# meta-pytorch/torchx

Hardware: AMD Instinct MI355X
Metric: tokens_per_second (higher is better)
Workload: dtype bf16; 1 GPU; model=llama3_8b, global_batch=4, seq_len=4096, parallelism=dp1

## Files before the change

torchx_amd/models/llama.py:

```python

from __future__ import annotations

from dataclasses import dataclass
from typing import Optional, Tuple

import torch
import torch.nn as nn

from torchx_amd import ops


@dataclass
class LlamaConfig:
    vocab_size: int = 128256
    hidden_size: int = 4096
    intermediate_size: int = 14336
    num_layers: int = 32
    num_heads: int = 32
    num_kv_heads: int = 8
    head_dim: int = 128
    max_seq_len: int = 8192
    rope_theta: float = 500000.0
    rms_eps: float = 1e-5
    tie_embeddings: bool = False

    @property
    def q_dim(self) -> int:
        return self.num_heads * self.head_dim

    @property
    def kv_dim(self) -> int:
        return self.num_kv_heads * self.head_dim


def llama3_8b() -> LlamaConfig:
    return LlamaConfig()


def llama_tiny(vocab: int = 512) -> LlamaConfig:
    return LlamaConfig(
        vocab_size=vocab, hidden_size=256, intermediate_size=512,
        num_layers=2, num_heads=4, num_kv_heads=2, head_dim=64,
        max_seq_len=256,
    )


def llama_gpu_tiny(vocab: int = 512) -> LlamaConfig:
    return LlamaConfig(
        vocab_size=vocab, hidden_size=2048, intermediate_size=4096,
        num_layers=2, num_heads=8, num_kv_heads=4, head_dim=128,
        max_seq_len=512,
    )


def _lin(mod: nn.Module, x: torch.Tensor) -> torch.Tensor:
    if type(mod) is nn.Linear and mod.bias is None and x.is_cuda:
        return ops.fast_linear(x, mod.weight)
    return mod(x)


def _new_linear(in_features: int, out_features: int,
                device: Optional[torch.device]) -> nn.Linear:
    if device is not None and torch.device(device).type == "cuda":
        return torch.nn.utils.skip_init(
            nn.Linear, in_features, out_features, bias=False,
            dtype=torch.bfloat16, device=device)
    return nn.Linear(in_features, out_features, bias=False,
                     dtype=torch.bfloat16)


class LlamaBlock(nn.Module):
    def __init__(self, cfg: LlamaConfig,
                 device: Optional[torch.device] = None):
        super().__init__()
        self.cfg = cfg
        h, qd, kvd = cfg.hidden_size, cfg.q_dim, cfg.kv_dim
        self.wqkv = _new_linear(h, qd + 2 * kvd, device)
        self.wo = _new_linear(qd, h, device)
        self.wgu = _new_linear(h, 2 * cfg.intermediate_size, device)
        self.wdown = _new_linear(cfg.intermediate_size, h, device)
        self.attn_norm = nn.Parameter(torch.ones(h, dtype=torch.bfloat16))
        self.mlp_norm = nn.Parameter(torch.ones(h, dtype=torch.bfloat16))

    def forward(self, x: torch.Tensor, cos: torch.Tensor,
                sin: torch.Tensor, delta: Optional[torch.Tensor] = None
                ) -> Tuple[torch.Tensor, torch.Tensor]:
        cfg = self.cfg
        B, S, H = x.shape
        if delta is None:
            xn = ops.rmsnorm(x, self.attn_norm, cfg.rms_eps)
        else:
            x, xn = ops.add_rmsnorm(x, delta, self.attn_norm, cfg.rms_eps)
        qkv = _lin(self.wqkv, xn)
        attn = ops.fused_attention_qkv(
            qkv, cos, sin, cfg.num_heads, cfg.num_kv_heads, causal=True
        )
        x, xn = ops.add_rmsnorm(
            x, _lin(self.wo, attn.reshape(B, S, cfg.q_dim)), self.mlp_norm,
            cfg.rms_eps)
        return x, _lin(self.wdown, ops.swiglu_packed(_lin(self.wgu, xn)))


class LlamaModel(nn.Module):

    def __init__(self, cfg: LlamaConfig, device: Optional[torch.device] = None):
        super().__init__()
        self.cfg = cfg
        factory = {"dtype": torch.bfloat16, "device": device}
        self.embed = nn.Embedding(cfg.vocab_size, cfg.hidden_size, **factory)
        self.blocks = nn.ModuleList(
            [LlamaBlock(cfg, device) for _ in range(cfg.num_layers)]
        )
        self.final_norm = nn.Parameter(
            torch.ones(cfg.hidden_size, dtype=torch.bfloat16)
        )
        self.lm_head = _new_linear(cfg.hidden_size, cfg.vocab_size, device)
        if cfg.tie_embeddings:
            self.lm_head.weight = self.embed.weight
        cos, sin = ops.rope_tables(cfg.max_seq_len, cfg.head_dim,
                                   cfg.rope_theta, device=device)
        self.register_buffer("rope_cos", cos, persistent=False)
        self.register_buffer("rope_sin", sin, persistent=False)
        if device is not None:
            self.to(device)
        self.apply(self._init_weights)

    def _init_weights(self, m: nn.Module) -> None:
        std = 0.02
        if isinstance(m, nn.Linear):
            nn.init.normal_(m.weight, mean=0.0, std=std)
        elif isinstance(m, nn.Embedding):
            nn.init.normal_(m.weight, mean=0.0, std=std)

    def forward_hidden(self, tokens: torch.Tensor) -> torch.Tensor:
        x = self.embed(tokens)
        cos, sin = self.rope_cos, self.rope_sin
        delta = None
        for blk in self.blocks:
            x, delta = blk(x, cos, sin, delta)
        if delta is None:
            return ops.rmsnorm(x, self.final_norm, self.cfg.rms_eps)
        return ops.add_rmsnorm(x, delta, self.final_norm,
                               self.cfg.rms_eps)[1]

    def forward(self, tokens: torch.Tensor,
                targets: Optional[torch.Tensor] = None) -> torch.Tensor:
        x = self.forward_hidden(tokens)
        if targets is None:
            return self.lm_head(x)
        return ops.fused_linear_cross_entropy(
            x, self.lm_head.weight, targets
        )

    def num_params(self) -> int:
        return sum(p.numel() for p in self.parameters())
```

torchx_amd/ops/__init__.py:

```python

from __future__ import annotations

import importlib.util
import math
from pathlib import Path
from typing import Optional, Tuple

import torch

from . import reference

_SO = Path(__file__).resolve().parent / "_hip_ops.so"
_hip = None
_load_err: Optional[str] = None


def _load():
    global _hip, _load_err
    if _hip is not None:
        return _hip
    if not _SO.exists():
        _load_err = f"{_SO} not built (run torchx_amd/ops/build.py)"
        return None
    try:
# ... 109 lines not shown
        return dx, None, None, None


def rope(x: torch.Tensor, cos: torch.Tensor, sin: torch.Tensor) -> torch.Tensor:
    heads = x.shape[2]
    if _on_gpu(x):
        return _RoPE.apply(x, cos, sin, heads)
    return reference.rope(x, cos, sin)




class _SwiGLU(torch.autograd.Function):
    @staticmethod
    def forward(ctx, g: torch.Tensor, u: torch.Tensor):
        ctx.save_for_backward(g, u)
        return hip_ops().swiglu_fwd(g.contiguous(), u.contiguous())

    @staticmethod
    def backward(ctx, dout: torch.Tensor):
        g, u = ctx.saved_tensors
        dg, du = hip_ops().swiglu_bwd(dout.contiguous(), g, u)
        return dg, du


def swiglu(g: torch.Tensor, u: torch.Tensor) -> torch.Tensor:
    if _on_gpu(g):
        return _SwiGLU.apply(g, u)
    return reference.swiglu(g, u)




class _CrossEntropy(torch.autograd.Function):
    @staticmethod
    def forward(ctx, logits: torch.Tensor, targets: torch.Tensor):
        V = logits.shape[-1]
        logits2d = logits.contiguous().view(-1, V)
        loss, lse = hip_ops().ce_fwd(logits2d, targets.contiguous().view(-1))
        ctx.save_for_backward(logits2d, targets, lse)
        ctx.orig_shape = logits.shape
        return loss.mean()

    @staticmethod
    def backward(ctx, gout: torch.Tensor):
        logits2d, targets, lse = ctx.saved_tensors
        T = logits2d.shape[0]
        gscale = (gout.float() / T).expand(T).contiguous()
        dlogits = hip_ops().ce_bwd(logits2d, targets.view(-1), lse, gscale)
        return dlogits.view(ctx.orig_shape), None


def cross_entropy(logits: torch.Tensor, targets: torch.Tensor) -> torch.Tensor:
    if _on_gpu(logits):
        return _CrossEntropy.apply(logits, targets)
    return reference.cross_entropy(logits, targets)




class _FusedLinearCE(torch.autograd.Function):
    @staticmethod
    def forward(ctx, x2: torch.Tensor, w: torch.Tensor,
                targets: torch.Tensor, chunk: int):
        hip = hip_ops()
        T, H = x2.shape
        dx = torch.empty_like(x2)
        single = T <= chunk
        dw_acc = None if single else torch.zeros_like(w, dtype=torch.float32)
        loss_sum = torch.zeros((), device=x2.device, dtype=torch.float32)
        inv_t = 1.0 / T
        gscale = torch.full((min(chunk, T),), inv_t, device=x2.device,
                            dtype=torch.float32)
        wt = (hip.transpose_bf16(w)
              if w.shape[0] % 64 == 0 and w.shape[1] % 64 == 0 else None)
        for s in range(0, T, chunk):
            e = min(T, s + chunk)
            x_c = x2[s:e]
            t_c = targets[s:e].contiguous()
            logits_c = x_c @ w.t()
            loss_c, lse_c = hip.ce_fwd(logits_c, t_c)
            loss_sum += loss_c.sum()
            dlog_c = hip.ce_bwd(logits_c, t_c, lse_c, gscale[:e - s])
            if wt is not None:
                torch.matmul(dlog_c, wt.t(), out=dx[s:e])
            else:
                torch.matmul(dlog_c, w, out=dx[s:e])
            if single:
                dw_acc = dlog_c.t() @ x_c
            else:
                dw_acc += dlog_c.t() @ x_c
        ctx.save_for_backward(dx, dw_acc)
        return loss_sum * inv_t

    @staticmethod
    def backward(ctx, gout: torch.Tensor):
        dx, dw_acc = ctx.saved_tensors
        if dw_acc.dtype == dx.dtype:
            dw = dw_acc * gout.to(dx.dtype)
        else:
            dw = (dw_acc * gout.to(torch.float32)).to(dx.dtype)
        dx = dx * gout.to(dx.dtype)
        return dx, dw, None, None


def fused_linear_cross_entropy(
    x: torch.Tensor, w: torch.Tensor, targets: torch.Tensor,
    chunk: int = 16384,
) -> torch.Tensor:
    H = x.shape[-1]
    x2 = x.reshape(-1, H)
    t = targets.reshape(-1)
    if _on_gpu(x):
        if torch.is_grad_enabled() and (x.requires_grad or w.requires_grad):
            return _FusedLinearCE.apply(x2.contiguous(), w, t, chunk)
        hip = hip_ops()
        x2 = x2.contiguous()
        T = x2.shape[0]
        loss_sum = torch.zeros((), device=x.device, dtype=torch.float32)
        for s in range(0, T, chunk):
            e = min(T, s + chunk)
            loss_c, _ = hip.ce_fwd(x2[s:e] @ w.t(), t[s:e].contiguous())
            loss_sum += loss_c.sum()
        return loss_sum / T
    return reference.cross_entropy(x2 @ w.t(), t)




class _FlashAttention(torch.autograd.Function):
    @staticmethod
    def forward(ctx, q: torch.Tensor, k: torch.Tensor, v: torch.Tensor,
                causal: bool, scale: float):
        o, lse = hip_ops().attn_fwd(
            q.contiguous(), k.contiguous(), v.contiguous(), scale, causal
        )
        ctx.save_for_backward(q, k, v, o, lse)
        ctx.causal = causal
        ctx.scale = scale
        return o

    @staticmethod
    def backward(ctx, dout: torch.Tensor):
        q, k, v, o, lse = ctx.saved_tensors
        dq, dk, dv = hip_ops().attn_bwd(
            q, k, v, o, dout.contiguous(), lse, ctx.scale, ctx.causal
        )
        return dq, dk, dv, None, None


def set_attn_bwd_dq_mode(mode: str) -> None:
    hip_ops().set_attn_bwd_dq_mode(mode)


def get_attn_bwd_dq_mode() -> str:
    return hip_ops().get_attn_bwd_dq_mode()


def set_attn_bwd_dkv_impl(impl: str) -> None:
    hip_ops().set_attn_bwd_dkv_impl(impl)


def get_attn_bwd_dkv_impl() -> str:
    return hip_ops().get_attn_bwd_dkv_impl()


def set_attn_fwd_map(name: str) -> None:
    hip_ops().set_attn_fwd_map(name)


def get_attn_fwd_map() -> str:
    return hip_ops().get_attn_fwd_map()


def flash_attention(
    q: torch.Tensor, k: torch.Tensor, v: torch.Tensor,
    causal: bool = True, scale: Optional[float] = None,
) -> torch.Tensor:
    if scale is None:
        scale = 1.0 / math.sqrt(q.shape[-1])
    if _on_gpu(q):
        return _FlashAttention.apply(q, k, v, causal, scale)
    return reference.attention(q, k, v, causal=causal, scale=scale)




def adamw_step(
    p32: torch.Tensor, p16: torch.Tensor, grad: torch.Tensor,
    m: torch.Tensor, v: torch.Tensor, *, lr: float, beta1: float = 0.9,
    beta2: float = 0.95, eps: float = 1e-8, weight_decay: float = 0.1,
    step: int = 1,
) -> None:
    if p32.is_cuda:
        hip_ops().adamw_step(p32, p16, grad, m, v, lr, beta1, beta2, eps,
                             weight_decay, step)
    else:
        reference.adamw_step(p32, p16, grad, m, v, lr=lr, beta1=beta1,
                             beta2=beta2, eps=eps, weight_decay=weight_decay,
                             step=step)


def mfma_probe(a: torch.Tensor, b: torch.Tensor) -> torch.Tensor:
    return hip_ops().mfma_probe(a, b)




class _FastLinear(torch.autograd.Function):
    @staticmethod
    def forward(ctx, x: torch.Tensor, w: torch.Tensor):
        ctx.save_for_backward(x, w)
        return x @ w.t()

    @staticmethod
    def backward(ctx, dy: torch.Tensor):
        x, w = ctx.saved_tensors
        hip = hip_ops()
        wt = hip.transpose_bf16(w)
        dy2 = dy.reshape(-1, dy.shape[-1]).contiguous()
        x2 = x.reshape(-1, x.shape[-1])
        dx = (dy2 @ wt.t()).view_as(x)
        M, N = dy2.shape
        via_t = N <= 8192 and M % 64 == 0 and N % 64 == 0
        wg = w.grad if w.is_leaf else None
        if wg is not None and wg.is_contiguous():
            a = hip.transpose_bf16(dy2) if via_t else dy2.t()
            if getattr(w, "_wgrad_fresh", False):
                torch.matmul(a, x2, out=wg)
                w._wgrad_fresh = False
            else:
                wg.addmm_(a, x2)
            from torchx_amd.parallel.ddp import grad_ready

            grad_ready(w)
            return dx, None
        dw = (hip.transpose_bf16(dy2) @ x2) if via_t else (dy2.t() @ x2)
        return dx, dw


def fast_linear(x: torch.Tensor, w: torch.Tensor) -> torch.Tensor:
    if (x.is_cuda and w.dtype == torch.bfloat16
            and w.shape[0] % 64 == 0 and w.shape[1] % 64 == 0):
        return _FastLinear.apply(x, w)
    return torch.nn.functional.linear(x, w)




class _FusedAttentionQKV(torch.autograd.Function):
    @staticmethod
    def forward(ctx, qkv: torch.Tensor, cos: torch.Tensor, sin: torch.Tensor,
                Hq: int, Hkv: int, causal: bool, scale: float):
        hip = hip_ops()
        roped = hip.rope_qkv(qkv.contiguous(), cos, sin, Hq, Hkv, 1.0, False)
        o, lse = hip.attn_fwd_qkv(roped, Hq, Hkv, scale, causal)
        ctx.save_for_backward(roped, o, lse, cos, sin)
        ctx.dims = (Hq, Hkv, causal, scale)
        return o

    @staticmethod
    def backward(ctx, dout: torch.Tensor):
        roped, o, lse, cos, sin = ctx.saved_tensors
        Hq, Hkv, causal, scale = ctx.dims
        hip = hip_ops()
        dqkv = hip.attn_bwd_qkv(roped, o, dout.contiguous(), lse, Hq, Hkv,
                                scale, causal)
        hip.rope_qkv(dqkv, cos, sin, Hq, Hkv, -1.0, True)
        return dqkv, None, None, None, None, None, None


def fused_attention_qkv(
    qkv: torch.Tensor, cos: torch.Tensor, sin: torch.Tensor,
    Hq: int, Hkv: int, causal: bool = True,
    scale: Optional[float] = None,
) -> torch.Tensor:
    D = qkv.shape[-1] // (Hq + 2 * Hkv)
    if scale is None:
        scale = 1.0 / math.sqrt(D)
    if _on_gpu(qkv):
        return _FusedAttentionQKV.apply(qkv, cos, sin, Hq, Hkv, causal, scale)
    B, S, _ = qkv.shape
    q, k, v = qkv.split([Hq * D, Hkv * D, Hkv * D], dim=-1)
    q = reference.rope(q.reshape(B, S, Hq, D), cos, sin)
    k = reference.rope(k.reshape(B, S, Hkv, D), cos, sin)
    return reference.attention(q, k, v.reshape(B, S, Hkv, D),
                               causal=causal, scale=scale)


class _SwiGLUPacked(torch.autograd.Function):
    @staticmethod
    def forward(ctx, gu: torch.Tensor):
        gu = gu.contiguous()
        ctx.save_for_backward(gu)
        return hip_ops().swiglu_gu_fwd(gu)

    @staticmethod
    def backward(ctx, dout: torch.Tensor):
        (gu,) = ctx.saved_tensors
        return hip_ops().swiglu_gu_bwd(dout.contiguous(), gu)


def swiglu_packed(gu: torch.Tensor) -> torch.Tensor:
    if _on_gpu(gu):
        return _SwiGLUPacked.apply(gu)
    g, u = gu.chunk(2, dim=-1)
    return reference.swiglu(g, u)




def decode_attention(q: torch.Tensor, kcache: torch.Tensor,
                     vcache: torch.Tensor, length: int,
                     scale: Optional[float] = None) -> torch.Tensor:
    if scale is None:
        scale = 1.0 / math.sqrt(q.shape[-1])
    if _on_gpu(q):
        return hip_ops().decode_attn(q.contiguous(), kcache, vcache,
                                     length, scale)
    return reference.decode_attention(q, kcache, vcache, length, scale)


def rmsnorm_res(x: torch.Tensor, res: Optional[torch.Tensor],
                w: torch.Tensor, eps: float = 1e-5):
    if _on_gpu(x):
        s, y = hip_ops().rmsnorm_res(x.contiguous(),
                                     res.contiguous() if res is not None
                                     else None, w.contiguous(), eps)
        return s, y
    s = x if res is None else (x + res)
    return s, reference.rmsnorm(s, w, eps)


def decode_rope_cache(qkv: torch.Tensor, kcache: torch.Tensor,
                      vcache: torch.Tensor, cos: torch.Tensor,
                      sin: torch.Tensor, pos,
                      num_heads: int) -> torch.Tensor:
    B = qkv.shape[0]
    Hkv, D = kcache.shape[2], kcache.shape[3]
    if _on_gpu(qkv):
        if isinstance(pos, torch.Tensor):
            return hip_ops().decode_rope_cache(qkv.contiguous(), kcache,
                                               vcache, cos, sin, 0, pos)
        return hip_ops().decode_rope_cache(qkv.contiguous(), kcache, vcache,
                                           cos, sin, int(pos), None)
    q, k, v = qkv.split([num_heads * D, Hkv * D, Hkv * D], dim=-1)
    q = q.reshape(B, 1, num_heads, D)
    k = k.reshape(B, 1, Hkv, D)
    v = v.reshape(B, 1, Hkv, D)
    if isinstance(pos, torch.Tensor) and pos.numel() > 1:
        outs = []
        for b in range(B):
            p = int(pos[b].item())
            cs, sn = cos[p:p + 1], sin[p:p + 1]
            outs.append(rope(q[b:b + 1].contiguous(), cs, sn))
            kcache[b, p:p + 1] = rope(k[b:b + 1].contiguous(), cs, sn)[0]
            vcache[b, p:p + 1] = v[b]
        return torch.cat(outs, dim=0).reshape(B, num_heads, D)
    p = int(pos.item()) if isinstance(pos, torch.Tensor) else int(pos)
    cs, sn = cos[p:p + 1], sin[p:p + 1]
    q = rope(q.contiguous(), cs, sn)
    k = rope(k.contiguous(), cs, sn)
    kcache[:, p:p + 1] = k
    vcache[:, p:p + 1] = v
    return q.reshape(B, num_heads, D)


def decode_linear_swiglu(x: torch.Tensor, w: torch.Tensor) -> torch.Tensor:
    x2 = x.reshape(-1, x.shape[-1])
    M, K = x2.shape
    if _on_gpu(x) and M <= 8 and K % 512 == 0 and w.shape[0] % 2 == 0 \
            and w.dtype == torch.bfloat16 and w.is_contiguous():
        out = hip_ops().gemv_swiglu_bf16(x2.contiguous(), w)
    else:
        gu = x2 @ w.t()
        g, u = gu.chunk(2, dim=-1)
        out = torch.nn.functional.silu(g.float()).to(u.dtype) * u
    return out.reshape(*x.shape[:-1], w.shape[0] // 2)


def decode_attention_dev(q: torch.Tensor, kcache: torch.Tensor,
                         vcache: torch.Tensor, pos: torch.Tensor,
                         scale: Optional[float] = None) -> torch.Tensor:
    if scale is None:
        scale = 1.0 / math.sqrt(q.shape[-1])
    if _on_gpu(q):
        return hip_ops().decode_attn_dev(q.contiguous(), kcache, vcache,
                                         pos.contiguous(), scale)
    if pos.numel() == 1:
        return reference.decode_attention(q, kcache, vcache,
# ... 162 lines not shown
```

torchx_amd/ops/csrc/bindings.cpp:

```cpp
#include <torch/extension.h>
#include <c10/hip/HIPStream.h>

#include <hip/hip_runtime.h>

extern "C" {
void rope_launch(const void*, void*, const void*, const void*, long, int, int,
                 int, float, hipStream_t);
void swiglu_fwd_launch(const void*, const void*, void*, long, hipStream_t);
void swiglu_bwd_launch(const void*, const void*, const void*, void*, void*,
                       long, hipStream_t);
void rmsnorm_fwd_launch(const void*, const void*, void*, void*, long, int,
                        float, hipStream_t);
void rmsnorm_bwd_launch(const void*, const void*, const void*, const void*,
                        const void*, void*, void*, void*, long, int,
                        hipStream_t);
long rmsnorm_bwd_dw_chunks(long);
void adamw_launch(void*, void*, const void*, void*, void*, long, float, float,
                  float, float, float, float, float, hipStream_t);
void ce_fwd_launch(const void*, const void*, void*, void*, long, int,
                   hipStream_t);
void ce_bwd_launch(const void*, const void*, const void*, const void*, void*,
                   long, int, hipStream_t);
void attn_fwd_launch(const void*, const void*, const void*, void*, void*, int,
                     int, int, int, float, int, long, long, hipStream_t);
void attn_bwd_launch(const void*, const void*, const void*, const void*,
                     const void*, const void*, void*, void*, void*, void*,
                     void*, int, int, int, int, float, int, long, long, long,
                     long, hipStream_t);
long attn_bwd_ds_bytes(int, int, int, int);
int attn_bwd_dkv_impl_get();
void attn_bwd_dkv_impl_set(int);
int attn_fwd_map_get();
void attn_fwd_map_set(int);
void rope_qkv_launch(const void*, void*, const void*, const void*, long, int,
                     long, int, float, hipStream_t);
void swiglu_gu_fwd_launch(const void*, void*, long, long, hipStream_t);
void swiglu_gu_bwd_launch(const void*, const void*, void*, long, long,
                          hipStream_t);
void mfma_probe_launch(const void*, const void*, void*, hipStream_t);
void mfma_probe_tr_launch(const void*, const void*, void*, void*,
                          hipStream_t);
void fp8_cast_transpose_launch(const void*, void*, void*, void*,
                               const void*, long, long, int, hipStream_t);
void transpose_bf16_launch(const void*, void*, long, long, hipStream_t);
void decode_attn_launch(const void*, const void*, const void*, void*,
                        const void*, int, int, int, int, int, int, float,
                        hipStream_t);
void gemv_bf16_launch(const void*, const void*, void*, int, int, int,
                      hipStream_t);
void decode_attn_split_launch(const void*, const void*, const void*, void*,
                              void*, void*, const void*, int, int, int, int,
                              int, int, int, float, hipStream_t);
void decode_rope_cache_launch(const void*, void*, void*, void*, const void*,
                              const void*, const void*, int, int, int, int,
                              int, int, hipStream_t);
void rmsnorm_res_launch(const void*, const void*, const void*, void*, void*,
                        void*, long, int, float, hipStream_t);
void gemv_swiglu_launch(const void*, const void*, void*, int, int, int,
                        hipStream_t);
void paged_decode_attn_launch(const void*, const void*, const void*, void*,
                              void*, void*, const void*, const void*, int,
                              int, int, int, int, int, int, float,
                              hipStream_t);
void paged_decode_rope_cache_launch(const void*, void*, void*, void*,
                                    const void*, const void*, const void*,
                                    const void*, int, int, int, int, int,
                                    int, int, hipStream_t);
void paged_prefill_attn_launch(const void*, const void*, const void*, void*,
                               const void*, const void*, int, int, int, int,
                               int, int, int, float, hipStream_t);
void paged_prefill_attn_ragged_launch(const void*, const void*, const void*,
                                      void*, const void*, const void*,
                                      const void*, int, int, int, int, int,
                                      int, int, int, float, hipStream_t);
void paged_prefill_rope_cache_launch(const void*, void*, void*, void*,
                                     const void*, const void*, const void*,
                                     const void*, long, int, int, long, int,
                                     hipStream_t);
}

namespace {

hipStream_t cur_stream() {
  return c10::hip::getCurrentHIPStream().stream();
}

void check_bf16(const at::Tensor& t, const char* name) {
  TORCH_CHECK(t.is_cuda(), name, " must be on GPU");
  TORCH_CHECK(t.scalar_type() == at::kBFloat16, name, " must be bf16");
  TORCH_CHECK(t.is_contiguous(), name, " must be contiguous");
}

void check_f32(const at::Tensor& t, const char* name) {
  TORCH_CHECK(t.is_cuda(), name, " must be on GPU");
  TORCH_CHECK(t.scalar_type() == at::kFloat, name, " must be f32");
  TORCH_CHECK(t.is_contiguous(), name, " must be contiguous");
}

}

std::vector<at::Tensor> rmsnorm_fwd(at::Tensor x, at::Tensor w, double eps) {
  check_bf16(x, "x");
  check_bf16(w, "w");
  const long H = x.size(-1);
  TORCH_CHECK(H % 2048 == 0 && H <= 8192, "rmsnorm: H must be k*2048, <=8192");
  const long rows = x.numel() / H;
  auto y = at::empty_like(x);
  auto invrms = at::empty({rows}, x.options().dtype(at::kFloat));
  rmsnorm_fwd_launch(x.data_ptr(), w.data_ptr(), y.data_ptr(),
                     invrms.data_ptr(), rows, (int)H, (float)eps,
                     cur_stream());
  return {y, invrms};
}

std::vector<at::Tensor> rmsnorm_bwd(at::Tensor dy, at::Tensor x, at::Tensor w,
                                    at::Tensor invrms,
                                    c10::optional<at::Tensor> dres) {
  check_bf16(dy, "dy");
  check_bf16(x, "x");
  check_bf16(w, "w");
  check_f32(invrms, "invrms");
// ... 184 lines not shown
                  cur_stream());
  return {dq, dk, dv};
}

std::vector<at::Tensor> attn_fwd_qkv(at::Tensor qkv, long Hq, long Hkv,
                                     double scale, bool causal) {
  check_bf16(qkv, "qkv");
  const int B = qkv.size(0), S = qkv.size(1);
  const long rs = (Hq + 2 * Hkv) * 128;
  TORCH_CHECK(qkv.size(2) == rs, "qkv last dim mismatch");
  auto o = at::empty({B, S, Hq, 128}, qkv.options());
  auto lse = at::empty({B, Hq, S}, qkv.options().dtype(at::kFloat));
  const unsigned short* base = (const unsigned short*)qkv.data_ptr();
  attn_fwd_launch(base, base + Hq * 128, base + (Hq + Hkv) * 128,
                  o.data_ptr(), lse.data_ptr(), B, S, (int)Hq, (int)Hkv,
                  (float)scale, causal ? 1 : 0, rs, rs, cur_stream());
  return {o, lse};
}

at::Tensor attn_bwd_qkv(at::Tensor qkv, at::Tensor o, at::Tensor dout,
                        at::Tensor lse, long Hq, long Hkv, double scale,
                        bool causal) {
  check_bf16(dout, "dout");
  const int B = qkv.size(0), S = qkv.size(1);
  const long rs = (Hq + 2 * Hkv) * 128;
  auto dqkv = at::empty_like(qkv);
  auto delta = at::empty({B, Hq, S}, qkv.options().dtype(at::kFloat));
  auto ds = alloc_ds_scratch(qkv, B, S, (int)Hq, causal);
  const unsigned short* base = (const unsigned short*)qkv.data_ptr();
  unsigned short* dbase = (unsigned short*)dqkv.data_ptr();
  attn_bwd_launch(base, base + Hq * 128, base + (Hq + Hkv) * 128,
                  o.data_ptr(), dout.data_ptr(), lse.data_ptr(),
                  delta.data_ptr(), dbase, dbase + Hq * 128,
                  dbase + (Hq + Hkv) * 128,
                  ds.defined() ? ds.data_ptr() : nullptr, B, S, (int)Hq,
                  (int)Hkv, (float)scale, causal ? 1 : 0, rs, rs, rs, rs,
                  cur_stream());
  return dqkv;
}

at::Tensor rope_qkv(at::Tensor x, at::Tensor cos_t, at::Tensor sin_t,
                    long Hq, long Hkv, double sign, bool inplace) {
  check_bf16(x, "x");
  check_f32(cos_t, "cos");
  check_f32(sin_t, "sin");
  const int B = x.size(0), S = x.size(1);
  const long rs = (Hq + 2 * Hkv) * 128;
  TORCH_CHECK(x.size(2) == rs, "qkv last dim mismatch");
  at::Tensor y = inplace ? x : at::empty_like(x);
  rope_qkv_launch(x.data_ptr(), y.data_ptr(), cos_t.data_ptr(),
                  sin_t.data_ptr(), (long)B * S, (int)(Hq + Hkv), rs, S,
                  (float)sign, cur_stream());
  if (!inplace) {
    const long v0 = (Hq + Hkv) * 128;
    y.narrow(2, v0, Hkv * 128).copy_(x.narrow(2, v0, Hkv * 128));
  }
  return y;
}

at::Tensor swiglu_gu_fwd(at::Tensor gu) {
  check_bf16(gu, "gu");
  const long twoI = gu.size(-1);
  TORCH_CHECK(twoI % 16 == 0, "gu last dim must be 2I, I % 8 == 0");
  const long I = twoI / 2;
  const long rows = gu.numel() / twoI;
  auto sizes = gu.sizes().vec();
  sizes.back() = I;
  auto out = at::empty(sizes, gu.options());
  swiglu_gu_fwd_launch(gu.data_ptr(), out.data_ptr(), rows, I, cur_stream());
  return out;
}

at::Tensor swiglu_gu_bwd(at::Tensor dout, at::Tensor gu) {
  check_bf16(dout, "dout");
  const long twoI = gu.size(-1);
  const long I = twoI / 2;
  const long rows = gu.numel() / twoI;
  auto dgu = at::empty_like(gu);
  swiglu_gu_bwd_launch(dout.data_ptr(), gu.data_ptr(), dgu.data_ptr(), rows,
                       I, cur_stream());
  return dgu;
}

std::vector<at::Tensor> fp8_cast_transpose(at::Tensor x, at::Tensor scale,
                                           bool e5m2) {
  check_bf16(x, "x");
  check_f32(scale, "scale");
  const long C = x.size(-1);
  const long R = x.numel() / C;
  TORCH_CHECK(R % 8 == 0 && C % 8 == 0, "fp8 cast: dims must be 8-aligned");
  auto dt = e5m2 ? at::kFloat8_e5m2 : at::kFloat8_e4m3fn;
  auto out = at::empty({R, C}, x.options().dtype(dt));
  auto out_t = at::empty({C, R}, x.options().dtype(dt));
  auto amax = at::zeros({1}, x.options().dtype(at::kFloat));
  fp8_cast_transpose_launch(x.data_ptr(), out.data_ptr(), out_t.data_ptr(),
                            amax.data_ptr(), scale.data_ptr(), R, C,
                            e5m2 ? 1 : 0, cur_stream());
  return {out, out_t, amax};
}

at::Tensor transpose_bf16(at::Tensor x) {
  check_bf16(x, "x");
  TORCH_CHECK(x.dim() == 2, "transpose_bf16: 2D only");
  const long R = x.size(0), C = x.size(1);
  TORCH_CHECK(R % 64 == 0 && C % 64 == 0,
              "transpose_bf16: dims must be multiples of 64");
  auto out = at::empty({C, R}, x.options());
  transpose_bf16_launch(x.data_ptr(), out.data_ptr(), R, C, cur_stream());
  return out;
}

at::Tensor decode_attn(at::Tensor q, at::Tensor kc, at::Tensor vc, long L,
                       double scale) {
  check_bf16(q, "q");
  check_bf16(kc, "kc");
  check_bf16(vc, "vc");
  const int B = q.size(0), Hq = q.size(1);
  const int T = kc.size(1), Hkv = kc.size(2);
  TORCH_CHECK(q.size(2) == 128 && kc.size(3) == 128, "head_dim must be 128");
  TORCH_CHECK(L >= 1 && L <= T, "invalid cache length");
  TORCH_CHECK(Hq % Hkv == 0, "GQA group mismatch");
  auto o = at::empty_like(q);
  const int split = std::max(1, std::min(16, 512 / (B * Hq)));
  if (split > 1) {
    auto ml = at::empty({(long)B * Hq * split * 2},
                        q.options().dtype(at::kFloat));
    auto oacc = at::empty({(long)B * Hq * split * 128},
                          q.options().dtype(at::kFloat));
    decode_attn_split_launch(q.data_ptr(), kc.data_ptr(), vc.data_ptr(),
                             ml.data_ptr(), oacc.data_ptr(), o.data_ptr(),
                             nullptr, B, Hq, Hkv, T, (int)L, split, 0,
                             (float)scale, cur_stream());
  } else {
    decode_attn_launch(q.data_ptr(), kc.data_ptr(), vc.data_ptr(),
                       o.data_ptr(), nullptr, B, Hq, Hkv, T, (int)L, 0,
                       (float)scale, cur_stream());
  }
  return o;
}

at::Tensor decode_attn_dev(at::Tensor q, at::Tensor kc, at::Tensor vc,
                           at::Tensor pos, double scale) {
  check_bf16(q, "q");
  const int B = q.size(0), Hq = q.size(1);
  TORCH_CHECK(pos.scalar_type() == at::kInt &&
                  (pos.numel() == 1 || pos.numel() == B),
              "pos must be an int32 scalar or [B] tensor on device");
  TORCH_CHECK(pos.is_contiguous(), "pos must be contiguous");
  const int per_row = pos.numel() == B && B > 1 ? 1 : 0;
  const int T = kc.size(1), Hkv = kc.size(2);
  auto o = at::empty_like(q);
  const int split = std::max(1, std::min(16, 512 / (B * Hq)));
  if (split > 1) {
    auto ml = at::empty({(long)B * Hq * split * 2},
                        q.options().dtype(at::kFloat));
    auto oacc = at::empty({(long)B * Hq * split * 128},
                          q.options().dtype(at::kFloat));
    decode_attn_split_launch(q.data_ptr(), kc.data_ptr(), vc.data_ptr(),
                             ml.data_ptr(), oacc.data_ptr(), o.data_ptr(),
                             pos.data_ptr(), B, Hq, Hkv, T, 0, split,
                             per_row, (float)scale, cur_stream());
  } else {
    decode_attn_launch(q.data_ptr(), kc.data_ptr(), vc.data_ptr(),
                       o.data_ptr(), pos.data_ptr(), B, Hq, Hkv, T, 0,
                       per_row, (float)scale, cur_stream());
  }
// ... 252 lines not shown
  TORCH_CHECK(H % 2048 == 0 && H <= 8192, "rmsnorm: H must be k*2048, <=8192");
  const long R = x.numel() / H;
  auto y = at::empty_like(x);
  at::Tensor s = x;
  const void* rp = nullptr;
  void* sp = nullptr;
  if (res.has_value()) {
    check_bf16(*res, "res");
    TORCH_CHECK(res->sizes() == x.sizes(), "res shape mismatch");
    s = at::empty_like(x);
    rp = res->data_ptr();
    sp = s.data_ptr();
  }
  rmsnorm_res_launch(x.data_ptr(), rp, w.data_ptr(), sp, y.data_ptr(),
                     nullptr, R, (int)H, (float)eps, cur_stream());
  return {s, y};
}

std::vector<at::Tensor> add_rmsnorm_fwd(at::Tensor x, at::Tensor delta,
                                        at::Tensor w, double eps) {
  check_bf16(x, "x");
  check_bf16(delta, "delta");
  check_bf16(w, "w");
  const long H = x.size(-1);
  TORCH_CHECK(H % 2048 == 0 && H <= 8192, "rmsnorm: H must be k*2048, <=8192");
  TORCH_CHECK(delta.sizes() == x.sizes(), "delta shape mismatch");
  TORCH_CHECK(w.numel() == H, "w size mismatch");
  const long R = x.numel() / H;
  auto s = at::empty_like(x);
  auto y = at::empty_like(x);
  auto invrms = at::empty({R}, x.options().dtype(at::kFloat));
  rmsnorm_res_launch(x.data_ptr(), delta.data_ptr(), w.data_ptr(),
                     s.data_ptr(), y.data_ptr(), invrms.data_ptr(), R, (int)H,
                     (float)eps, cur_stream());
  return {s, y, invrms};
}

std::vector<at::Tensor> mfma_probe_tr(at::Tensor a, at::Tensor b) {
  check_bf16(a, "a");
  check_bf16(b, "b");
  TORCH_CHECK(a.size(0) == 32 && a.size(1) == 16, "a must be [32,16]");
  TORCH_CHECK(b.size(0) == 16 && b.size(1) == 32, "b must be [16,32]");
  auto c = at::empty({32, 32}, a.options().dtype(at::kFloat));
  auto raw = at::empty({64, 8}, a.options());
  mfma_probe_tr_launch(a.data_ptr(), b.data_ptr(), c.data_ptr(),
                       raw.data_ptr(), cur_stream());
  return {c, raw};
}

at::Tensor mfma_probe(at::Tensor a, at::Tensor b) {
  check_bf16(a, "a");
  check_bf16(b, "b");
  TORCH_CHECK(a.size(0) == 32 && a.size(1) == 16, "a must be [32,16]");
  TORCH_CHECK(b.size(0) == 16 && b.size(1) == 32, "b must be [16,32]");
  auto c = at::empty({32, 32}, a.options().dtype(at::kFloat));
  mfma_probe_launch(a.data_ptr(), b.data_ptr(), c.data_ptr(), cur_stream());
  return c;
}

PYBIND11_MODULE(TORCH_EXTENSION_NAME, m) {
  m.def("rmsnorm_fwd", &rmsnorm_fwd);
  m.def("rmsnorm_bwd", &rmsnorm_bwd, py::arg("dy"), py::arg("x"),
        py::arg("w"), py::arg("invrms"), py::arg("dres") = c10::nullopt);
  m.def("add_rmsnorm_fwd", &add_rmsnorm_fwd);
  m.def("rope", &rope);
  m.def("swiglu_fwd", &swiglu_fwd);
  m.def("swiglu_bwd", &swiglu_bwd);
  m.def("adamw_step", &adamw_step);
  m.def("ce_fwd", &ce_fwd);
  m.def("ce_bwd", &ce_bwd);
  m.def("attn_fwd", &attn_fwd);
  m.def("attn_bwd", &attn_bwd);
  m.def("set_attn_bwd_dq_mode", &set_attn_bwd_dq_mode);
  m.def("get_attn_bwd_dq_mode", &get_attn_bwd_dq_mode);
  m.def("set_attn_bwd_dkv_impl", &set_attn_bwd_dkv_impl);
  m.def("get_attn_bwd_dkv_impl", &get_attn_bwd_dkv_impl);
  m.def("set_attn_fwd_map", &set_attn_fwd_map);
  m.def("get_attn_fwd_map", &get_attn_fwd_map);
  m.def("attn_fwd_qkv", &attn_fwd_qkv);
  m.def("attn_bwd_qkv", &attn_bwd_qkv);
  m.def("rope_qkv", &rope_qkv);
  m.def("swiglu_gu_fwd", &swiglu_gu_fwd);
  m.def("swiglu_gu_bwd", &swiglu_gu_bwd);
  m.def("fp8_cast_transpose", &fp8_cast_transpose);
  m.def("mfma_probe", &mfma_probe);
  m.def("mfma_probe_tr", &mfma_probe_tr);
  m.def("transpose_bf16", &transpose_bf16);
  m.def("decode_attn", &decode_attn);
  m.def("decode_attn_dev", &decode_attn_dev);
  m.def("gemv_bf16", &gemv_bf16);
  m.def("gemv_swiglu_bf16", &gemv_swiglu_bf16);
  m.def("decode_rope_cache", &decode_rope_cache,
        py::arg("qkv"), py::arg("kc"), py::arg("vc"), py::arg("cos"),
        py::arg("sin"), py::arg("pos") = 0,
        py::arg("pos_dev") = c10::nullopt);
  m.def("paged_decode_attn", &paged_decode_attn);
  m.def("paged_decode_rope_cache", &paged_decode_rope_cache);
  m.def("paged_prefill_attn", &paged_prefill_attn);
  m.def("paged_prefill_attn_ragged", &paged_prefill_attn_ragged);
  m.def("paged_prefill_rope_cache", &paged_prefill_rope_cache);
  m.def("rmsnorm_res", &rmsnorm_res,
        py::arg("x"), py::arg("res"), py::arg("w"), py::arg("eps"));
}
```

torchx_amd/ops/csrc/elementwise.hip:

```cpp
#include "common.h"

__global__ void rope_fwdbwd_kernel(
    const unsigned short* __restrict__ x,
    unsigned short* __restrict__ y,
    const float* __restrict__ cos_t,
    const float* __restrict__ sin_t,
    long np4,
    int half_d,
    int heads,
    int seq_len,
    float sign) {
  typedef unsigned short us4 __attribute__((ext_vector_type(4)));
  typedef float f4 __attribute__((ext_vector_type(4)));
  for (long p4 = grid_stride_begin(); p4 < np4; p4 += grid_stride()) {
    long p = p4 * 4;
    long row = p / half_d;
    int i = (int)(p % half_d);
    int pos = (int)((row / heads) % seq_len);
    const long base = row * (2L * half_d);
    us4 u1 = *(const us4*)(x + base + i);
    us4 u2 = *(const us4*)(x + base + half_d + i);
    f4 c = *(const f4*)(cos_t + (long)pos * half_d + i);
    f4 s = *(const f4*)(sin_t + (long)pos * half_d + i);
    us4 o1, o2;
// ... 101 lines not shown
  if (grid == 0) grid = 1;
  hipLaunchKernelGGL(swiglu_bwd_kernel, dim3((int)grid), dim3(block), 0,
                     stream, (const unsigned short*)dout,
                     (const unsigned short*)g, (const unsigned short*)u,
                     (unsigned short*)dg, (unsigned short*)du, n8);
}

__global__ void rope_qkv_kernel(
    const unsigned short* __restrict__ x,
    unsigned short* __restrict__ y,
    const float* __restrict__ cos_t,
    const float* __restrict__ sin_t,
    long np4,
    int nh,
    long row_stride,
    int seq_len,
    float sign) {
  typedef unsigned short us4 __attribute__((ext_vector_type(4)));
  typedef float f4 __attribute__((ext_vector_type(4)));
  const int half_d = 64;
  const long hp4 = (long)blockIdx.x * blockDim.x + threadIdx.x;
  if (hp4 >= (long)nh * 16) return;
  const int h = (int)(hp4 >> 4);
  const int i = (int)(hp4 & 15) * 4;
  const long rows = np4 / ((long)nh * 16);
  for (long row = blockIdx.y; row < rows; row += gridDim.y) {
    const int pos = (int)(row % seq_len);
    const long base = row * row_stride + (long)h * 128;
    us4 u1 = *(const us4*)(x + base + i);
    us4 u2 = *(const us4*)(x + base + half_d + i);
    f4 c = *(const f4*)(cos_t + (long)pos * half_d + i);
    f4 s = *(const f4*)(sin_t + (long)pos * half_d + i);
    us4 o1, o2;
    #pragma unroll
    for (int j = 0; j < 4; ++j) {
      float x1 = bf16_to_f32(u1[j]);
      float x2 = bf16_to_f32(u2[j]);
      o1[j] = f32_to_bf16(fmaf(x1, c[j], -sign * s[j] * x2));
      o2[j] = f32_to_bf16(fmaf(x2, c[j], sign * s[j] * x1));
    }
    *(us4*)(y + base + i) = o1;
    *(us4*)(y + base + half_d + i) = o2;
  }
}

extern "C" void rope_qkv_launch(
    const void* x, void* y, const void* cos_t, const void* sin_t,
    long rows, int nh, long row_stride, int seq_len, float sign,
    hipStream_t stream) {
  const long np4 = rows * nh * 16;
  const int block = 256;
  const int gx = (int)(((long)nh * 16 + block - 1) / block);
  const int gy = (int)((rows < 65535) ? (rows > 0 ? rows : 1) : 65535);
  hipLaunchKernelGGL(rope_qkv_kernel, dim3(gx, gy), dim3(block), 0,
                     stream, (const unsigned short*)x, (unsigned short*)y,
                     (const float*)cos_t, (const float*)sin_t, np4, nh,
                     row_stride, seq_len, sign);
}

__global__ void swiglu_gu_fwd_kernel(
    const unsigned short* __restrict__ gu,
    unsigned short* __restrict__ out,
    long rows,
    long i8) {
  const long c8 = (long)blockIdx.x * blockDim.x + threadIdx.x;
  if (c8 >= i8) return;
  for (long row = blockIdx.y; row < rows; row += gridDim.y) {
    const long base = row * 2 * i8 * 8 + c8 * 8;
    ushort8 gv = *(const ushort8*)(gu + base);
    ushort8 uv = *(const ushort8*)(gu + base + i8 * 8);
    ushort8 ov;
    #pragma unroll
    for (int j = 0; j < 8; ++j) {
      float gf = bf16_to_f32(gv[j]);
      float uf = bf16_to_f32(uv[j]);
      float sig =
          1.0f / (1.0f + __builtin_amdgcn_exp2f(-1.44269504f * gf));
      ov[j] = f32_to_bf16(gf * sig * uf);
    }
    *(ushort8*)(out + (row * i8 + c8) * 8) = ov;
  }
}

__global__ void swiglu_gu_bwd_kernel(
    const unsigned short* __restrict__ dout,
    const unsigned short* __restrict__ gu,
    unsigned short* __restrict__ dgu,
    long rows, long i8) {
  const long c8 = (long)blockIdx.x * blockDim.x + threadIdx.x;
  if (c8 >= i8) return;
  for (long row = blockIdx.y; row < rows; row += gridDim.y) {
    const long base = row * 2 * i8 * 8 + c8 * 8;
    ushort8 dov = *(const ushort8*)(dout + (row * i8 + c8) * 8);
    ushort8 gv = *(const ushort8*)(gu + base);
    ushort8 uv = *(const ushort8*)(gu + base + i8 * 8);
    ushort8 dgv, duv;
    #pragma unroll
    for (int j = 0; j < 8; ++j) {
      float dof = bf16_to_f32(dov[j]);
      float gf = bf16_to_f32(gv[j]);
      float uf = bf16_to_f32(uv[j]);
      float sig =
          1.0f / (1.0f + __builtin_amdgcn_exp2f(-1.44269504f * gf));
      float silu = gf * sig;
      dgv[j] = f32_to_bf16(dof * uf * sig * (1.0f + gf * (1.0f - sig)));
      duv[j] = f32_to_bf16(dof * silu);
    }
    *(ushort8*)(dgu + base) = dgv;
    *(ushort8*)(dgu + base + i8 * 8) = duv;
  }
}

extern "C" void swiglu_gu_fwd_launch(const void* gu, void* out, long rows,
                                     long I, hipStream_t stream) {
  const long i8 = I / 8;
  const int block = 256;
  const int gx = (int)((i8 + block - 1) / block);
  const int gy = (int)((rows < 65535) ? (rows > 0 ? rows : 1) : 65535);
  hipLaunchKernelGGL(swiglu_gu_fwd_kernel, dim3(gx, gy), dim3(block), 0,
                     stream, (const unsigned short*)gu, (unsigned short*)out,
                     rows, i8);
}

extern "C" void swiglu_gu_bwd_launch(const void* dout, const void* gu,
                                     void* dgu, long rows, long I,
                                     hipStream_t stream) {
  const long i8 = I / 8;
  const int block = 256;
  const int gx = (int)((i8 + block - 1) / block);
  const int gy = (int)((rows < 65535) ? (rows > 0 ? rows : 1) : 65535);
  hipLaunchKernelGGL(swiglu_gu_bwd_kernel, dim3(gx, gy), dim3(block), 0,
                     stream, (const unsigned short*)dout,
                     (const unsigned short*)gu, (unsigned short*)dgu, rows,
                     i8);
}

#define TP 64

__global__ void __launch_bounds__(256)
transpose_bf16_kernel(const unsigned short* __restrict__ in,
                      unsigned short* __restrict__ out, int R, int C) {
  __shared__ unsigned short tile[TP][TP + 1];
  const int tile_r = blockIdx.y * TP;
  const int tile_c = blockIdx.x * TP;

  #pragma unroll
  for (int pass = 0; pass < 2; ++pass) {
    const int idx = pass * 2048 + threadIdx.x * 8;
    const int r = idx / TP;
    const int c = idx % TP;
    ushort8 v = *(const ushort8*)(in + (long)(tile_r + r) * C + tile_c + c);
    #pragma unroll
    for (int j = 0; j < 8; ++j) tile[r][c + j] = v[j];
  }
  __syncthreads();
  #pragma unroll
  for (int pass = 0; pass < 2; ++pass) {
    const int idx = pass * 2048 + threadIdx.x * 8;
    const int oc = idx / TP;
    const int orr = idx % TP;
    ushort8 v;
    #pragma unroll
    for (int j = 0; j < 8; ++j) v[j] = tile[orr + j][oc];
    *(ushort8*)(out + (long)(tile_c + oc) * R + tile_r + orr) = v;
  }
}

extern "C" void transpose_bf16_launch(const void* in, void* out, long R,
                                      long C, hipStream_t stream) {
  hipLaunchKernelGGL(transpose_bf16_kernel,
                     dim3((int)(C / TP), (int)(R / TP)), dim3(256), 0,
                     stream, (const unsigned short*)in, (unsigned short*)out,
                     (int)R, (int)C);
}
```

Measured before the change: 22010 tokens/s.

## Fuse SwiGLU backward with transpose and reorder transpose block tiling

```diff
diff --git a/torchx_amd/models/llama.py b/torchx_amd/models/llama.py
--- a/torchx_amd/models/llama.py
+++ b/torchx_amd/models/llama.py
@@ -69,6 +69,12 @@
                      dtype=torch.bfloat16)
 
 
+def _lin_swiglu(mod: nn.Module, x: torch.Tensor) -> torch.Tensor:
+    if type(mod) is nn.Linear and mod.bias is None and x.is_cuda:
+        return ops.linear_swiglu(x, mod.weight)
+    return ops.swiglu_packed(mod(x))
+
+
 class LlamaBlock(nn.Module):
     def __init__(self, cfg: LlamaConfig,
                  device: Optional[torch.device] = None):
@@ -98,7 +104,7 @@
         x, xn = ops.add_rmsnorm(
             x, _lin(self.wo, attn.reshape(B, S, cfg.q_dim)), self.mlp_norm,
             cfg.rms_eps)
-        return x, _lin(self.wdown, ops.swiglu_packed(_lin(self.wgu, xn)))
+        return x, _lin(self.wdown, _lin_swiglu(self.wgu, xn))
 
 
 class LlamaModel(nn.Module):
diff --git a/torchx_amd/ops/__init__.py b/torchx_amd/ops/__init__.py
--- a/torchx_amd/ops/__init__.py
+++ b/torchx_amd/ops/__init__.py
@@ -215,6 +215,7 @@
             loss_c, lse_c = hip.ce_fwd(logits_c, t_c)
             loss_sum += loss_c.sum()
             dlog_c = hip.ce_bwd(logits_c, t_c, lse_c, gscale[:e - s])
+            del logits_c
             if wt is not None:
                 torch.matmul(dlog_c, wt.t(), out=dx[s:e])
             else:
@@ -223,6 +224,7 @@
                 dw_acc = dlog_c.t() @ x_c
             else:
                 dw_acc += dlog_c.t() @ x_c
+            del dlog_c
         ctx.save_for_backward(dx, dw_acc)
         return loss_sum * inv_t
 
@@ -354,22 +356,32 @@
         dy2 = dy.reshape(-1, dy.shape[-1]).contiguous()
         x2 = x.reshape(-1, x.shape[-1])
         dx = (dy2 @ wt.t()).view_as(x)
-        M, N = dy2.shape
-        via_t = N <= 8192 and M % 64 == 0 and N % 64 == 0
-        wg = w.grad if w.is_leaf else None
-        if wg is not None and wg.is_contiguous():
-            a = hip.transpose_bf16(dy2) if via_t else dy2.t()
-            if getattr(w, "_wgrad_fresh", False):
-                torch.matmul(a, x2, out=wg)
-                w._wgrad_fresh = False
-            else:
-                wg.addmm_(a, x2)
-            from torchx_amd.parallel.ddp import grad_ready
-
-            grad_ready(w)
-            return dx, None
-        dw = (hip.transpose_bf16(dy2) @ x2) if via_t else (dy2.t() @ x2)
-        return dx, dw
+        return dx, _wgrad(hip, w, dy2, x2)
+
+
+def _wgrad(hip, w: torch.Tensor, dy2: torch.Tensor, x2: torch.Tensor,
+           dyt: Optional[torch.Tensor] = None) -> Optional[torch.Tensor]:
+    M, N = dy2.shape
+    K = x2.shape[1]
+    aligned = M % 64 == 0 and N % 64 == 0
+    both_t = aligned and N > 8192 and K % 64 == 0
+    if both_t or (aligned and N <= 8192):
+        a = dyt if dyt is not None else hip.transpose_bf16(dy2)
+    else:
+        a = dy2.t()
+    b = hip.transpose_bf16(x2.contiguous()).t() if both_t else x2
+    wg = w.grad if w.is_leaf else None
+    if wg is not None and wg.is_contiguous():
+        if getattr(w, "_wgrad_fresh", False):
+            torch.matmul(a, b, out=wg)
+            w._wgrad_fresh = False
+        else:
+            wg.addmm_(a, b)
+        from torchx_amd.parallel.ddp import grad_ready
+
+        grad_ready(w)
+        return None
+    return a @ b
 
 
 def fast_linear(x: torch.Tensor, w: torch.Tensor) -> torch.Tensor:
@@ -439,6 +451,38 @@
         return _SwiGLUPacked.apply(gu)
     g, u = gu.chunk(2, dim=-1)
     return reference.swiglu(g, u)
+
+
+class _LinearSwiGLU(torch.autograd.Function):
+
+    @staticmethod
+    def forward(ctx, x: torch.Tensor, w: torch.Tensor):
+        hip = hip_ops()
+        gu = x @ w.t()
+        ctx.save_for_backward(x, w, gu)
+        return hip.swiglu_gu_fwd(gu)
+
+    @staticmethod
+    def backward(ctx, dout: torch.Tensor):
+        x, w, gu = ctx.saved_tensors
+        hip = hip_ops()
+        dout = dout.contiguous()
+        gu2 = gu.view(-1, gu.shape[-1])
+        if gu2.shape[0] % 64 == 0 and gu2.shape[1] % 128 == 0:
+            dgu2, dgut = hip.swiglu_gu_bwd_t(dout.view(-1, dout.shape[-1]),
+                                             gu2)
+        else:
+            dgu2, dgut = hip.swiglu_gu_bwd(dout, gu2), None
+        wt = hip.transpose_bf16(w)
+        dx = (dgu2 @ wt.t()).view_as(x)
+        return dx, _wgrad(hip, w, dgu2, x.reshape(-1, x.shape[-1]), dgut)
+
+
+def linear_swiglu(x: torch.Tensor, w: torch.Tensor) -> torch.Tensor:
+    if (x.is_cuda and w.dtype == torch.bfloat16 and x.dtype == w.dtype
+            and w.shape[0] % 64 == 0 and w.shape[1] % 64 == 0):
+        return _LinearSwiGLU.apply(x, w)
+    return swiglu_packed(fast_linear(x, w))
 
 
 
diff --git a/torchx_amd/ops/csrc/bindings.cpp b/torchx_amd/ops/csrc/bindings.cpp
--- a/torchx_amd/ops/csrc/bindings.cpp
+++ b/torchx_amd/ops/csrc/bindings.cpp
@@ -37,6 +37,8 @@
 void swiglu_gu_fwd_launch(const void*, void*, long, long, hipStream_t);
 void swiglu_gu_bwd_launch(const void*, const void*, void*, long, long,
                           hipStream_t);
+void swiglu_gu_bwd_t_launch(const void*, const void*, void*, void*, long,
+                            long, hipStream_t);
 void mfma_probe_launch(const void*, const void*, void*, hipStream_t);
 void mfma_probe_tr_launch(const void*, const void*, void*, void*,
                           hipStream_t);
@@ -387,6 +389,24 @@
   return dgu;
 }
 
+std::vector<at::Tensor> swiglu_gu_bwd_t(at::Tensor dout, at::Tensor gu) {
+  check_bf16(dout, "dout");
+  check_bf16(gu, "gu");
+  const long twoI = gu.size(-1);
+  const long I = twoI / 2;
+  const long rows = gu.numel() / twoI;
+  TORCH_CHECK(twoI % 2 == 0 && I % 64 == 0 && rows % 64 == 0 && rows > 0 &&
+                  (rows / 64) * (I / 64) < (1L << 31),
+              "swiglu_gu_bwd_t: rows and I must be multiples of 64");
+  TORCH_CHECK(dout.numel() == rows * I && dout.size(-1) == I,
+              "swiglu_gu_bwd_t: dout must be [rows, I]");
+  auto dgu = at::empty_like(gu);
+  auto dguT = at::empty({twoI, rows}, gu.options());
+  swiglu_gu_bwd_t_launch(dout.data_ptr(), gu.data_ptr(), dgu.data_ptr(),
+                         dguT.data_ptr(), rows, I, cur_stream());
+  return {dgu, dguT};
+}
+
 std::vector<at::Tensor> fp8_cast_transpose(at::Tensor x, at::Tensor scale,
                                            bool e5m2) {
   check_bf16(x, "x");
@@ -805,6 +825,7 @@
   m.def("rope_qkv", &rope_qkv);
   m.def("swiglu_gu_fwd", &swiglu_gu_fwd);
   m.def("swiglu_gu_bwd", &swiglu_gu_bwd);
+  m.def("swiglu_gu_bwd_t", &swiglu_gu_bwd_t);
   m.def("fp8_cast_transpose", &fp8_cast_transpose);
   m.def("mfma_probe", &mfma_probe);
   m.def("mfma_probe_tr", &mfma_probe_tr);
diff --git a/torchx_amd/ops/csrc/elementwise.hip b/torchx_amd/ops/csrc/elementwise.hip
--- a/torchx_amd/ops/csrc/elementwise.hip
+++ b/torchx_amd/ops/csrc/elementwise.hip
@@ -207,6 +207,22 @@
   }
 }
 
+__device__ __forceinline__ void swiglu_gu_bwd8(
+    const ushort8& dov, const ushort8& gv, const ushort8& uv,
+    ushort8& dgv, ushort8& duv) {
+  #pragma unroll
+  for (int j = 0; j < 8; ++j) {
+    float dof = bf16_to_f32(dov[j]);
+    float gf = bf16_to_f32(gv[j]);
+    float uf = bf16_to_f32(uv[j]);
+    float sig =
+        1.0f / (1.0f + __builtin_amdgcn_exp2f(-1.44269504f * gf));
+    float silu = gf * sig;
+    dgv[j] = f32_to_bf16(dof * uf * sig * (1.0f + gf * (1.0f - sig)));
+    duv[j] = f32_to_bf16(dof * silu);
+  }
+}
+
 __global__ void swiglu_gu_bwd_kernel(
     const unsigned short* __restrict__ dout,
     const unsigned short* __restrict__ gu,
@@ -220,17 +236,7 @@
     ushort8 gv = *(const ushort8*)(gu + base);
     ushort8 uv = *(const ushort8*)(gu + base + i8 * 8);
     ushort8 dgv, duv;
-    #pragma unroll
-    for (int j = 0; j < 8; ++j) {
-      float dof = bf16_to_f32(dov[j]);
-      float gf = bf16_to_f32(gv[j]);
-      float uf = bf16_to_f32(uv[j]);
-      float sig =
-          1.0f / (1.0f + __builtin_amdgcn_exp2f(-1.44269504f * gf));
-      float silu = gf * sig;
-      dgv[j] = f32_to_bf16(dof * uf * sig * (1.0f + gf * (1.0f - sig)));
-      duv[j] = f32_to_bf16(dof * silu);
-    }
+    swiglu_gu_bwd8(dov, gv, uv, dgv, duv);
     *(ushort8*)(dgu + base) = dgv;
     *(ushort8*)(dgu + base + i8 * 8) = duv;
   }
@@ -262,12 +268,25 @@
 
 #define TP 64
 
+#define TGROUP 32
+
+__device__ __forceinline__ void tile_of_block(int bid, int nrow, int ncol,
+                                              int& rt, int& ct) {
+  const int grp = bid / (TGROUP * ncol);
+  const int rem = bid - grp * (TGROUP * ncol);
+  const int glen = min(TGROUP, nrow - grp * TGROUP);
+  rt = grp * TGROUP + rem % glen;
+  ct = rem / glen;
+}
+
 __global__ void __launch_bounds__(256)
 transpose_bf16_kernel(const unsigned short* __restrict__ in,
                       unsigned short* __restrict__ out, int R, int C) {
   __shared__ unsigned short tile[TP][TP + 1];
-  const int tile_r = blockIdx.y * TP;
-  const int tile_c = blockIdx.x * TP;
+  int rt, ct;
+  tile_of_block((int)blockIdx.x, R / TP, C / TP, rt, ct);
+  const int tile_r = rt * TP;
+  const int tile_c = ct * TP;
 
   #pragma unroll
   for (int pass = 0; pass < 2; ++pass) {
@@ -291,10 +310,71 @@
   }
 }
 
+__global__ void __launch_bounds__(256)
+swiglu_gu_bwd_t_kernel(const unsigned short* __restrict__ dout,
+                       const unsigned short* __restrict__ gu,
+                       unsigned short* __restrict__ dgu,
+                       unsigned short* __restrict__ dguT,
+                       long rows, long I) {
+  __shared__ unsigned short tg[TP][TP + 1];
+  __shared__ unsigned short tu[TP][TP + 1];
+  int rt, ct;
+  tile_of_block((int)blockIdx.x, (int)(rows / TP), (int)(I / TP), rt, ct);
+  const long tile_r = (long)rt * TP;
+  const long tile_c = (long)ct * TP;
+
+  #pragma unroll
+  for (int pass = 0; pass < 2; ++pass) {
+    const int idx = pass * 2048 + threadIdx.x * 8;
+    const int r = idx / TP;
+    const int c = idx % TP;
+    const long row = tile_r + r;
+    const long base = row * 2 * I + tile_c + c;
+    ushort8 dov = *(const ushort8*)(dout + row * I + tile_c + c);
+    ushort8 gv = *(const ushort8*)(gu + base);
+    ushort8 uv = *(const ushort8*)(gu + base + I);
+    ushort8 dgv, duv;
+    swiglu_gu_bwd8(dov, gv, uv, dgv, duv);
+    *(ushort8*)(dgu + base) = dgv;
+    *(ushort8*)(dgu + base + I) = duv;
+    #pragma unroll
+    for (int j = 0; j < 8; ++j) {
+      tg[r][c + j] = dgv[j];
+      tu[r][c + j] = duv[j];
+    }
+  }
+  __syncthreads();
+  #pragma unroll
+  for (int pass = 0; pass < 2; ++pass) {
+    const int idx = pass * 2048 + threadIdx.x * 8;
+    const int oc = idx / TP;
+    const int orr = idx % TP;
+    ushort8 vg, vu;
+    #pragma unroll
+    for (int j = 0; j < 8; ++j) {
+      vg[j] = tg[orr + j][oc];
+      vu[j] = tu[orr + j][oc];
+    }
+    const long o = (tile_c + oc) * rows + tile_r + orr;
+    *(ushort8*)(dguT + o) = vg;
+    *(ushort8*)(dguT + o + I * rows) = vu;
+  }
+}
+
+extern "C" void swiglu_gu_bwd_t_launch(const void* dout, const void* gu,
+                                       void* dgu, void* dguT, long rows,
+                                       long I, hipStream_t stream) {
+  hipLaunchKernelGGL(swiglu_gu_bwd_t_kernel,
+                     dim3((unsigned)((I / TP) * (rows / TP))), dim3(256), 0,
+                     stream, (const unsigned short*)dout,
+                     (const unsigned short*)gu, (unsigned short*)dgu,
+                     (unsigned short*)dguT, rows, I);
+}
+
 extern "C" void transpose_bf16_launch(const void* in, void* out, long R,
                                       long C, hipStream_t stream) {
   hipLaunchKernelGGL(transpose_bf16_kernel,
-                     dim3((int)(C / TP), (int)(R / TP)), dim3(256), 0,
+                     dim3((unsigned)((C / TP) * (R / TP))), dim3(256), 0,
                      stream, (const unsigned short*)in, (unsigned short*)out,
                      (int)R, (int)C);
 }
```

New measurement: 22820 tokens/s, median of 6. +3.7%, better.
